# caishiqing/voice-tts

Measured on AMD Instinct MI355X. Metric: audio_seconds_per_second, higher is better.
Workload: dtype bf16

## Files before the change

### include/ixtts_hip.h

```cpp
#ifndef IXTTS_HIP_H
#define IXTTS_HIP_H

#include <stddef.h>
#include <stdint.h>

#ifdef __cplusplus
extern "C" {
#endif

#define IXTTS_OK 0
#define IXTTS_ERR_ARG (-1)
#define IXTTS_ERR_HIP (-2)
#define IXTTS_ERR_STATE (-3)
#define IXTTS_ERR_NOMEM (-4)
#define IXTTS_ERR_NAME (-5)

const char* ixtts_version(void);
const char* ixtts_last_error(void);

int ixtts_aa_snake_f32(const float* x_dev, float* y_dev, const float* up12_dev, const float* down12_dev,
                       const float* log_alpha_dev, const float* log_beta_dev, int B, int C, int T, void* stream);

size_t ixtts_attn_full_workspace_bytes(int B, int H, int T);
int ixtts_attn_full_f32(const float* q_dev, const float* k_dev, const float* v_dev, float* out_dev, int B, int H, int T,
                        int head_dim, long stride_b, long stride_t, long stride_h, long ostride_b, long ostride_t,
                        long ostride_h, float scale, void* workspace_dev, size_t workspace_bytes, void* stream);

int ixtts_adaln_rmsnorm_f32(const float* x_dev, const float* wb_dev, const float* g_dev, float* out_dev, int B, int T, int H, float eps,
                            void* stream);
int ixtts_ln_modulate_f32(const float* x_dev, const float* shift_scale_dev, float* out_dev, int B, int T, int H, float eps, void* stream);
int ixtts_rope_qk_f32(float* qkv_dev, const float* cos_sin_dev, int B, int T, int H, int head_dim, void* stream);
int ixtts_swiglu_f32(const float* u_dev, float* out_dev, long rows, int F, void* stream);
int ixtts_wn_gate_f32(const float* a_dev, const float* g_dev, float* out_dev, int B, int C, int T, long g_stride, int g_offset, void* stream);
int ixtts_wn_gate_rows_f32(const float* a_dev, const float* g_dev, float* out_dev, long rows, int C, long rows_per_batch, int B, long g_stride,
                           int g_offset, void* stream);
int ixtts_reflect_halo_rows_f32(float* p_dev, int B, int T, int C, int left, int right, void* stream);

size_t ixtts_gemm_x6_packed_bytes(int N, int K);
int ixtts_gemm_x6_pack(const float* w_dev, void* packed_dev, int N, int K, void* stream);
long ixtts_gemm_x6_rows_padded(long rows);
int ixtts_gemm_x6_split(const float* a_dev, long lda, void* planes_dev, long rows, int K, void* stream);
int ixtts_gemm_x6_f32(const void* a_planes_dev, long rows_total, long row0, const void* packed_dev, const float* bias_dev, float* c_dev, long ldc,
                      int M, int N, int K, int accumulate, int tile, void* stream);

#define IXTTS_BIGVGAN_MAX_STAGES 8
#define IXTTS_BIGVGAN_MAX_RESK 4

typedef struct ixtts_bigvgan_cfg {
  int num_mels;
  int upsample_initial_channel;
  int n_stages;
  int upsample_rates[IXTTS_BIGVGAN_MAX_STAGES];
  int upsample_kernel_sizes[IXTTS_BIGVGAN_MAX_STAGES];
  int n_resblock_kernels;
  int resblock_kernel_sizes[IXTTS_BIGVGAN_MAX_RESK];
  int resblock_dilations[IXTTS_BIGVGAN_MAX_RESK][3];
  int max_frames;
  int fast_sin;
} ixtts_bigvgan_cfg;

typedef struct ixtts_bigvgan ixtts_bigvgan;

int ixtts_bigvgan_create(ixtts_bigvgan** out, const ixtts_bigvgan_cfg* cfg);
int ixtts_bigvgan_set_tensor(ixtts_bigvgan* h, const char* name, const float* data_host, const int64_t* shape, int ndim);
int ixtts_bigvgan_finalize(ixtts_bigvgan* h);
int ixtts_bigvgan_arena(ixtts_bigvgan* h, void** ptr_dev, size_t* bytes);
int ixtts_bigvgan_adopt_arena(ixtts_bigvgan* h);
int ixtts_bigvgan_forward(ixtts_bigvgan* h, const float* mel_dev, int B, int F, float* wav_dev, void* stream);
double ixtts_bigvgan_flops(const ixtts_bigvgan* h, int B, int F);
int ixtts_bigvgan_destroy(ixtts_bigvgan* h);

#define IXTTS_DTYPE_F32 0
#define IXTTS_DTYPE_BF16 1

typedef struct ixtts_gpt_cfg {
  int model_dim;
// ... 69 lines not shown
```

### voice-tts_amd/_lib.py

```python
import ctypes as C
import os

HERE = os.path.dirname(os.path.abspath(__file__))
LIB_PATH = os.environ.get("IXTTS_LIB") or os.path.join(HERE, "libixtts_hip.so")

MAX_STAGES = 8
MAX_RESK = 4


class BigVGANCfg(C.Structure):
    _fields_ = [
        ("num_mels", C.c_int), ("upsample_initial_channel", C.c_int), ("n_stages", C.c_int),
        ("upsample_rates", C.c_int * MAX_STAGES), ("upsample_kernel_sizes", C.c_int * MAX_STAGES),
        ("n_resblock_kernels", C.c_int), ("resblock_kernel_sizes", C.c_int * MAX_RESK),
        ("resblock_dilations", (C.c_int * 3) * MAX_RESK), ("max_frames", C.c_int), ("fast_sin", C.c_int),
    ]


class GptCfg(C.Structure):
    _fields_ = [
        ("model_dim", C.c_int), ("layers", C.c_int), ("heads", C.c_int), ("n_mel_codes", C.c_int),
        ("n_mel_pos", C.c_int), ("n_text_tokens", C.c_int), ("n_text_pos", C.c_int),
        ("start_mel_token", C.c_int), ("stop_mel_token", C.c_int), ("max_seq", C.c_int),
        ("max_batch", C.c_int), ("weight_dtype", C.c_int),
    ]


class SamplerCfg(C.Structure):
    _fields_ = [
        ("repetition_penalty", C.c_float), ("temperature", C.c_float), ("top_k", C.c_int),
        ("top_p", C.c_float), ("do_sample", C.c_int), ("suppress_stop", C.c_int), ("seed", C.c_uint64),
        ("typical_mass", C.c_float), ("length_penalty", C.c_float),
    ]


_P = C.c_void_p
SYMBOLS = {
    "ixtts_version": (C.c_char_p, []),
    "ixtts_last_error": (C.c_char_p, []),
    "ixtts_aa_snake_f32": (C.c_int, [_P, _P, _P, _P, _P, _P, C.c_int, C.c_int, C.c_int, _P]),
    "ixtts_attn_full_workspace_bytes": (C.c_size_t, [C.c_int, C.c_int, C.c_int]),
    "ixtts_attn_full_f32": (C.c_int, [_P, _P, _P, _P, C.c_int, C.c_int, C.c_int, C.c_int, C.c_long, C.c_long, C.c_long, C.c_long, C.c_long,
                                      C.c_long, C.c_float, _P, C.c_size_t, _P]),
    "ixtts_adaln_rmsnorm_f32": (C.c_int, [_P, _P, _P, _P, C.c_int, C.c_int, C.c_int, C.c_float, _P]),
    "ixtts_ln_modulate_f32": (C.c_int, [_P, _P, _P, C.c_int, C.c_int, C.c_int, C.c_float, _P]),
    "ixtts_rope_qk_f32": (C.c_int, [_P, _P, C.c_int, C.c_int, C.c_int, C.c_int, _P]),
    "ixtts_swiglu_f32": (C.c_int, [_P, _P, C.c_long, C.c_int, _P]),
    "ixtts_wn_gate_f32": (C.c_int, [_P, _P, _P, C.c_int, C.c_int, C.c_int, C.c_long, C.c_int, _P]),
    "ixtts_wn_gate_rows_f32": (C.c_int, [_P, _P, _P, C.c_long, C.c_int, C.c_long, C.c_int, C.c_long, C.c_int, _P]),
    "ixtts_reflect_halo_rows_f32": (C.c_int, [_P, C.c_int, C.c_int, C.c_int, C.c_int, C.c_int, _P]),
    "ixtts_gemm_x6_packed_bytes": (C.c_size_t, [C.c_int, C.c_int]),
    "ixtts_gemm_x6_pack": (C.c_int, [_P, _P, C.c_int, C.c_int, _P]),
    "ixtts_gemm_x6_rows_padded": (C.c_long, [C.c_long]),
    "ixtts_gemm_x6_split": (C.c_int, [_P, C.c_long, _P, C.c_long, C.c_int, _P]),
    "ixtts_gemm_x6_f32": (C.c_int, [_P, C.c_long, C.c_long, _P, _P, _P, C.c_long, C.c_int, C.c_int, C.c_int, C.c_int, C.c_int, _P]),
    "ixtts_bigvgan_create": (C.c_int, [C.POINTER(_P), C.POINTER(BigVGANCfg)]),
    "ixtts_bigvgan_set_tensor": (C.c_int, [_P, C.c_char_p, _P, C.POINTER(C.c_int64), C.c_int]),
    "ixtts_bigvgan_finalize": (C.c_int, [_P]),
    "ixtts_bigvgan_arena": (C.c_int, [_P, C.POINTER(_P), C.POINTER(C.c_size_t)]),
    "ixtts_bigvgan_adopt_arena": (C.c_int, [_P]),
    "ixtts_bigvgan_forward": (C.c_int, [_P, _P, C.c_int, C.c_int, _P, _P]),
    "ixtts_bigvgan_flops": (C.c_double, [_P, C.c_int, C.c_int]),
    "ixtts_bigvgan_destroy": (C.c_int, [_P]),
    "ixtts_gpt_create": (C.c_int, [C.POINTER(_P), C.POINTER(GptCfg)]),
    "ixtts_gpt_set_tensor": (C.c_int, [_P, C.c_char_p, _P, C.POINTER(C.c_int64), C.c_int]),
    "ixtts_gpt_finalize": (C.c_int, [_P]),
    "ixtts_gpt_arena": (C.c_int, [_P, C.POINTER(_P), C.POINTER(C.c_size_t)]),
    "ixtts_gpt_adopt_arena": (C.c_int, [_P]),
    "ixtts_gpt_share_arena": (C.c_int, [_P, _P]),
    "ixtts_gpt_prefill": (C.c_int, [_P, C.c_int, _P, C.c_int, C.c_int, _P]),
    "ixtts_gpt_decode": (C.c_int, [_P, C.c_int, C.c_int, C.POINTER(SamplerCfg), _P]),
    "ixtts_gpt_read": (C.c_int, [_P, C.c_int, _P, C.c_int, C.POINTER(C.c_int), C.POINTER(C.c_int), _P]),
    "ixtts_gpt_read_logits": (C.c_int, [_P, C.c_int, _P, _P]),
    "ixtts_gpt_beam_begin": (C.c_int, [_P, C.c_int, _P]),
    "ixtts_gpt_beam_decode": (C.c_int, [_P, C.c_int, C.POINTER(SamplerCfg), _P]),
    "ixtts_gpt_beam_read": (C.c_int, [_P, C.c_int, _P, C.c_int, C.POINTER(C.c_int), C.POINTER(C.c_int), C.POINTER(C.c_float), _P, _P, _P, _P]),
    "ixtts_gpt_beam_force": (C.c_int, [_P, _P, C.c_int, _P]),
    "ixtts_gpt_beam_begin_group": (C.c_int, [_P, C.c_int, C.c_int, C.c_uint64, _P]),
    "ixtts_gpt_beam_park_group": (C.c_int, [_P, C.c_int, _P]),
    "ixtts_gpt_beam_decode_groups": (C.c_int, [_P, C.c_int, C.c_int, C.POINTER(SamplerCfg), _P]),
    "ixtts_gpt_beam_read_group": (C.c_int, [_P, C.c_int, C.c_int, _P, C.c_int, C.POINTER(C.c_int), C.POINTER(C.c_int), C.POINTER(C.c_float), _P, _P, _P, _P]),
    "ixtts_gpt_beam_force_group": (C.c_int, [_P, C.c_int, _P, C.c_int, _P]),
    "ixtts_gpt_read_probs": (C.c_int, [_P, C.c_int, _P, _P]),
    "ixtts_gpt_force_next": (C.c_int, [_P, C.c_int, C.c_int32, _P]),
    "ixtts_gpt_latent": (C.c_int, [_P, _P, C.c_int, _P, C.c_int, _P, _P]),
    "ixtts_gpt_bench_gemv": (C.c_int, [_P, C.c_int, C.c_int, C.c_int, _P]),
    "ixtts_gpt_step_bytes": (C.c_double, [_P, C.c_int, C.c_int]),
    "ixtts_gpt_max_batch": (C.c_int, []),
# ... 44 lines not shown
```

### voice-tts_amd/csrc/gemm_x6.hip

```cpp
#include "common.h"

namespace ixtts {

typedef float gx_f32x16 __attribute__((ext_vector_type(16)));
typedef __bf16 gx_bf16x8 __attribute__((ext_vector_type(8)));
typedef float gx_f32x4 __attribute__((ext_vector_type(4)));
typedef unsigned int gx_u32x4 __attribute__((ext_vector_type(4)));


__global__ void gemm_x6_pack_kernel(const float* __restrict__ w, uint4* __restrict__ out, int N, int K, int Npad) {
  const long total = (long)(K / 8) * Npad;
  for (long idx = blockIdx.x * (long)blockDim.x + threadIdx.x; idx < total; idx += (long)gridDim.x * blockDim.x) {
    const int n = (int)(idx % Npad);
    const int ko = (int)(idx / Npad);
    float v[8];
#pragma unroll
    for (int e = 0; e < 8; ++e) v[e] = n < N ? w[(long)n * K + ko * 8 + e] : 0.f;
    uint4 ph, pm, pl;
    split8_bf16x3(v, ph, pm, pl);
    const int g = ko >> 1, kh = ko & 1;
    uint4* base = out + ((long)g * 6) * Npad + n;
    base[(long)(0 * 2 + kh) * Npad] = ph;
    base[(long)(1 * 2 + kh) * Npad] = pm;
    base[(long)(2 * 2 + kh) * Npad] = pl;
  }
}

__global__ __launch_bounds__(256) void gemm_x6_split_kernel(const float* __restrict__ a, long lda, uint4* __restrict__ out, int M, int K, long Mpad) {
  __shared__ float tile[64][65];
  const int r0 = blockIdx.x * 64, k0 = blockIdx.y * 64;
  const int t = threadIdx.x;
#pragma unroll
  for (int i = 0; i < 4; ++i) {
    const int r = (t >> 4) + 16 * i, kq = t & 15;
    float4 v = make_float4(0.f, 0.f, 0.f, 0.f);
    if (r0 + r < M) v = *reinterpret_cast<const float4*>(a + (long)(r0 + r) * lda + k0 + 4 * kq);
    tile[r][4 * kq + 0] = v.x; tile[r][4 * kq + 1] = v.y; tile[r][4 * kq + 2] = v.z; tile[r][4 * kq + 3] = v.w;
  }
  __syncthreads();
#pragma unroll
  for (int u = 0; u < 2; ++u) {
    const int r = t & 63, o = (t >> 6) + 4 * u;
    float v[8];
#pragma unroll
    for (int e = 0; e < 8; ++e) v[e] = tile[r][o * 8 + e];
    uint4 ph, pm, pl;
    split8_bf16x3(v, ph, pm, pl);
    const int ko = (k0 >> 3) + o, g = ko >> 1, kh = ko & 1;
    uint4* base = out + ((long)g * 6) * Mpad + r0 + r;
    base[(long)(0 * 2 + kh) * Mpad] = ph;
    base[(long)(1 * 2 + kh) * Mpad] = pm;
    base[(long)(2 * 2 + kh) * Mpad] = pl;
  }
}

struct GemmX6Params {
  const uint4* Ap;
  long Mpad;
  long arow0;
  const uint4* Wp;
  const float* bias;
  float* C;
  long ldc;
  int M, N, Npad, K, accumulate, m_tiles, n_tiles;
  unsigned long long* dbg;
};


template <int MT, int NT, int NST, int DBG = 0>
__global__ __launch_bounds__(256, (NST * (MT + NT) * 6 * 64 * 16 <= 80 * 1024) ? 2 : 1) void gemm_x6_kernel(GemmX6Params p) {
  constexpr int BM = 64 * MT, BN = 64 * NT;
  constexpr int A_UNITS = 6 * BM, W_UNITS = 6 * BN, STAGE = A_UNITS + W_UNITS;
  constexpr int NDMA = (6 * (MT + NT)) / 4;
  static_assert((6 * (MT + NT)) % 4 == 0, "the copies are dealt evenly to the 4 waves");
  constexpr int D = NST - 1;
  extern __shared__ uint4 smem[];

  const int nwg = p.m_tiles * p.n_tiles;
  const int bid = blockIdx.x;
  const int xcd = bid & 7, idx = bid >> 3;
  const int qd = nwg >> 3, rm = nwg & 7;
  const int lin = (xcd < rm ? xcd * (qd + 1) : rm * (qd + 1) + (xcd - rm) * qd) + idx;
  const int m_tile = lin / p.n_tiles, n_tile = lin - m_tile * p.n_tiles;
  const int m0 = m_tile * BM, n0 = n_tile * BN;

  const int tid = threadIdx.x, lane = tid & 63, wave = tid >> 6;
  const int wm = wave >> 1, wn = wave & 1;
  const int l31 = lane & 31, lh = lane >> 5;

  gx_f32x16 acc[MT][NT];
#pragma unroll
  for (int i = 0; i < MT; ++i)
#pragma unroll
    for (int j = 0; j < NT; ++j)
#pragma unroll
      for (int r = 0; r < 16; ++r) acc[i][j][r] = 0.f;

  const uint4* asrc = p.Ap + p.arow0 + m0 + lane;
  const uint4* wsrc = p.Wp + n0 + lane;
  auto issue = [&](int s, uint4* st) {
#pragma unroll
    for (int q = 0; q < NDMA; ++q) {
      const int e = q * 4 + wave;
      if (e < 6 * MT) {
        const int run = e / MT, piece = e % MT;
        __builtin_amdgcn_global_load_lds((const __attribute__((address_space(1))) void*)(asrc + ((long)s * 6 + run) * p.Mpad + piece * 64),
                                         (__attribute__((address_space(3))) void*)(st + run * BM + piece * 64), 16, 0, 0);
      } else {
        const int e2 = e - 6 * MT, run = e2 / NT, piece = e2 % NT;
        __builtin_amdgcn_global_load_lds((const __attribute__((address_space(1))) void*)(wsrc + ((long)s * 6 + run) * p.Npad + piece * 64),
                                         (__attribute__((address_space(3))) void*)(st + A_UNITS + run * BN + piece * 64), 16, 0, 0);
      }
    }
  };

  const int steps = p.K >> 4;
  auto wg_stamp = [&](int k) {
    if constexpr (DBG == 3) {
      if (tid == 0) p.dbg[128 + (long)blockIdx.x * 4 + k] = __builtin_amdgcn_s_memrealtime();
    }
  };
  auto wait_younger = [&](int y) {
    if (y >= 2) asm volatile("s_waitcnt vmcnt(%0)" ::"n"(2 * NDMA) : "memory");
    else if (y == 1) asm volatile("s_waitcnt vmcnt(%0)" ::"n"(NDMA) : "memory");
    else asm volatile("s_waitcnt vmcnt(0)" ::: "memory");
  };
  static_assert(D >= 1 && D <= 3, "1..3 steps of copies in flight behind the one waited for");
  wg_stamp(0);
  for (int t = 0; t < D && t < steps; ++t) issue(t, smem + t * STAGE);
  wait_younger(min(D, steps) - 1);
  __builtin_amdgcn_s_barrier();
  asm volatile("" ::: "memory");
  wg_stamp(1);

  const unsigned base_addr = (unsigned)(uintptr_t)(const __attribute__((address_space(3))) void*)smem;
  int st_cur = 0, st_nxt = D % NST;
  for (int s = 0; s < steps; ++s) {
    auto stamp = [&](int k) {
      if constexpr (DBG == 3) {
// ... 37 lines not shown
              "=&v"(bf[1][0]), "=&v"(bf[1][1]), "=&v"(bf[2][0]), "=&v"(bf[2][1])
            : "v"(aaddr), "v"(waddr), "n"((0 * 2 * BM + 0) * 16), "n"((0 * 2 * BM + 32) * 16), "n"((1 * 2 * BM + 0) * 16), "n"((1 * 2 * BM + 32) * 16),
              "n"((2 * 2 * BM + 0) * 16), "n"((2 * 2 * BM + 32) * 16), "n"((0 * 2 * BN + 0) * 16), "n"((0 * 2 * BN + 32) * 16), "n"((1 * 2 * BN + 0) * 16),
              "n"((1 * 2 * BN + 32) * 16), "n"((2 * 2 * BN + 0) * 16), "n"((2 * 2 * BN + 32) * 16)
            : "memory");
      }
      stamp(2);
#pragma unroll
      for (int i = 0; i < MT; ++i)
#pragma unroll
        for (int j = 0; j < NT; ++j) {
          const gx_bf16x8 ah = __builtin_bit_cast(gx_bf16x8, af[0][i]), am = __builtin_bit_cast(gx_bf16x8, af[1][i]), al = __builtin_bit_cast(gx_bf16x8, af[2][i]);
          const gx_bf16x8 bh = __builtin_bit_cast(gx_bf16x8, bf[0][j]), bm = __builtin_bit_cast(gx_bf16x8, bf[1][j]), bl = __builtin_bit_cast(gx_bf16x8, bf[2][j]);
          acc[i][j] = __builtin_amdgcn_mfma_f32_32x32x16_bf16(al, bh, acc[i][j], 0, 0, 0);
          acc[i][j] = __builtin_amdgcn_mfma_f32_32x32x16_bf16(ah, bl, acc[i][j], 0, 0, 0);
          acc[i][j] = __builtin_amdgcn_mfma_f32_32x32x16_bf16(am, bm, acc[i][j], 0, 0, 0);
          acc[i][j] = __builtin_amdgcn_mfma_f32_32x32x16_bf16(am, bh, acc[i][j], 0, 0, 0);
          acc[i][j] = __builtin_amdgcn_mfma_f32_32x32x16_bf16(ah, bm, acc[i][j], 0, 0, 0);
          acc[i][j] = __builtin_amdgcn_mfma_f32_32x32x16_bf16(ah, bh, acc[i][j], 0, 0, 0);
        }
      if constexpr (DBG == 3) asm volatile("" ::"v"(acc[0][0][0]), "v"(acc[MT - 1][NT - 1][15]));
    }
    stamp(3);
    wait_younger(DBG == 1 ? 0 : max(0, min(D - 1, steps - s - 2)));
    stamp(4);
    __builtin_amdgcn_s_barrier();
    asm volatile("" ::: "memory");
    stamp(5);
    st_cur = st_cur + 1 == NST ? 0 : st_cur + 1;
    st_nxt = st_nxt + 1 == NST ? 0 : st_nxt + 1;
  }

  wg_stamp(2);
#pragma unroll
  for (int j = 0; j < NT; ++j) {
    const int col = n0 + wn * (32 * NT) + j * 32 + l31;
    const bool col_ok = col < p.N;
    const float bv = (p.bias != nullptr && col_ok) ? p.bias[col] : 0.f;
#pragma unroll
    for (int i = 0; i < MT; ++i) {
      const int rbase = m0 + wm * (32 * MT) + i * 32 + 4 * lh;
#pragma unroll
      for (int r = 0; r < 16; ++r) {
        const int row = rbase + (r & 3) + 8 * (r >> 2);
        if (col_ok && row < p.M) {
          float* c = p.C + (long)row * p.ldc + col;
          float v = acc[i][j][r] + bv;
          if (p.accumulate) v += *c;
          *c = v;
        }
      }
    }
  }
  if constexpr (DBG == 3) {
    asm volatile("s_waitcnt vmcnt(0)" ::: "memory");
    wg_stamp(3);
  }
}

template <int MT, int NT, int NST, int DBG = 0>
static int launch_gemm_x6(GemmX6Params p, hipStream_t st) {
  constexpr int BM = 64 * MT, BN = 64 * NT;
  constexpr size_t smem = (size_t)NST * (6 * BM + 6 * BN) * 16;
  static_assert(smem <= 160 * 1024, "LDS stages of this tile shape");
  p.m_tiles = ceil_div(p.M, BM);
  p.n_tiles = ceil_div(p.N, BN);
  IX_ARG((long)p.n_tiles * BN <= p.Npad, "gemm_x6: packed weights padded to %d features, the %d-wide tile needs %d", p.Npad, BN, p.n_tiles * BN);
  IX_ARG(p.arow0 + (long)p.m_tiles * BM <= p.Mpad, "gemm_x6: activation planes hold %ld rows, the %d-row tiles reach row %ld", p.Mpad, BM, p.arow0 + (long)p.m_tiles * BM);
  auto kern = gemm_x6_kernel<MT, NT, NST, DBG>;
  static bool done = false;
  if (!done) {
    IX_HIP(hipFuncSetAttribute((const void*)kern, hipFuncAttributeMaxDynamicSharedMemorySize, (int)smem));
    done = true;
  }
  hipLaunchKernelGGL(kern, dim3(p.m_tiles * p.n_tiles), dim3(256), smem, st, p);
  IX_HIP(hipGetLastError());
  return IXTTS_OK;
}

}

using namespace ixtts;

extern "C" size_t ixtts_gemm_x6_packed_bytes(int N, int K) {
  if (N <= 0 || K <= 0 || K % 64) return 0;
  const size_t Npad = (size_t)(N + 255) / 256 * 256;
  return (size_t)(K / 16) * 6 * Npad * 16;
}

extern "C" int ixtts_gemm_x6_pack(const float* w_dev, void* packed_dev, int N, int K, void* stream) {
  IX_ARG(w_dev && packed_dev && N > 0 && K > 0 && K % 64 == 0, "gemm_x6_pack: bad argument (K must be a multiple of 64)");
  const int Npad = (N + 255) / 256 * 256;
  const long total = (long)(K / 8) * Npad;
  hipLaunchKernelGGL(gemm_x6_pack_kernel, dim3((unsigned)std::min<long>((total + 255) / 256, 4096)), dim3(256), 0, (hipStream_t)stream, w_dev,
                     reinterpret_cast<uint4*>(packed_dev), N, K, Npad);
  IX_HIP(hipGetLastError());
  return IXTTS_OK;
}

extern "C" long ixtts_gemm_x6_rows_padded(long rows) { return rows <= 0 ? 0 : (rows + 255) / 256 * 256 + 256; }

extern "C" int ixtts_gemm_x6_split(const float* a_dev, long lda, void* planes_dev, long rows, int K, void* stream) {
  IX_ARG(a_dev && planes_dev && rows > 0 && K > 0 && K % 64 == 0, "gemm_x6_split: bad argument (K must be a multiple of 64)");
  IX_ARG(lda >= K && lda % 4 == 0 && (reinterpret_cast<uintptr_t>(a_dev) & 15) == 0, "gemm_x6_split: rows must be 16-byte aligned (lda %ld)", lda);
  const long Mpad = ixtts_gemm_x6_rows_padded(rows);
  hipLaunchKernelGGL(gemm_x6_split_kernel, dim3((unsigned)(Mpad / 64), K / 64), dim3(256), 0, (hipStream_t)stream, a_dev, lda,
                     reinterpret_cast<uint4*>(planes_dev), (int)rows, K, Mpad);
  IX_HIP(hipGetLastError());
  return IXTTS_OK;
}

extern "C" int ixtts_gemm_x6_f32(const void* a_planes_dev, long rows_total, long row0, const void* packed_dev, const float* bias_dev, float* c_dev,
                                 long ldc, int M, int N, int K, int accumulate, int tile, void* stream) {
  IX_ARG(a_planes_dev && packed_dev && c_dev && M > 0 && N > 0 && K > 0 && K % 64 == 0, "gemm_x6: bad argument (K must be a multiple of 64: the split pass works on 64-wide k blocks)");
  IX_ARG(ldc >= N && row0 >= 0 && row0 + M <= rows_total, "gemm_x6: rows [%ld, %ld) of %ld, ldc %ld", row0, row0 + M, rows_total, ldc);
  GemmX6Params p;
  p.Ap = reinterpret_cast<const uint4*>(a_planes_dev); p.Mpad = ixtts_gemm_x6_rows_padded(rows_total); p.arow0 = row0;
  p.Wp = reinterpret_cast<const uint4*>(packed_dev); p.bias = bias_dev; p.C = c_dev; p.ldc = ldc;
  p.M = M; p.N = N; p.Npad = (N + 255) / 256 * 256; p.K = K; p.accumulate = accumulate ? 1 : 0; p.m_tiles = p.n_tiles = 0;
  p.dbg = (tile == 32 || tile == 33) ? reinterpret_cast<unsigned long long*>(const_cast<float*>(bias_dev)) : nullptr;
  if (p.dbg) p.bias = nullptr;
  hipStream_t st = (hipStream_t)stream;
  if (tile == 0) {
    const long t42 = (long)ceil_div(M, 256) * ceil_div(N, 128);
    tile = t42 >= 140 ? 2 : 3;
  }
  switch (tile) {
    case 2: return launch_gemm_x6<4, 2, 2>(p, st);
    case 3: return launch_gemm_x6<2, 2, 3>(p, st);
    case 4: return launch_gemm_x6<4, 2, 4>(p, st);
    case 5: return launch_gemm_x6<2, 2, 4>(p, st);
    case 12: return launch_gemm_x6<4, 2, 2, 1>(p, st);
    case 22: return launch_gemm_x6<4, 2, 2, 2>(p, st);
    case 32: return launch_gemm_x6<4, 2, 2, 3>(p, st);
    case 33: return launch_gemm_x6<2, 2, 3, 3>(p, st);
  }
  set_error("gemm_x6: tile %d (0 auto; 2 / 3: 256x128 / 128x128, two workgroups per CU; 4 / 5: the same, one per CU with a 4-stage ring)", tile);
  return IXTTS_ERR_ARG;
}
```

### voice-tts_amd/gemm.py

```python
import ctypes as C

import torch

from . import _lib


class PackedLinear:

    __slots__ = ("N", "K", "packed", "bias")

    def __init__(self, weight, bias=None):
        assert weight.is_cuda and weight.dim() == 2 and weight.shape[1] % 64 == 0, tuple(weight.shape)
        w = weight.detach().to(torch.float32).contiguous()
        self.N, self.K = int(w.shape[0]), int(w.shape[1])
        nbytes = _lib.lib().ixtts_gemm_x6_packed_bytes(self.N, self.K)
        self.packed = torch.empty(nbytes, dtype=torch.uint8, device=w.device)
        with torch.cuda.device(w.device):
            _lib.check(_lib.lib().ixtts_gemm_x6_pack(w.data_ptr(), self.packed.data_ptr(), self.N, self.K, _lib.current_stream_ptr()), "ixtts_gemm_x6_pack")
            torch.cuda.current_stream().synchronize()
        self.bias = None if bias is None else bias.detach().to(w.device, torch.float32).contiguous()


class Planes:

# ... 15 lines not shown
    K = int(x.shape[-1])
    if x.dim() != 2:
        x = x.reshape(-1, K) if x.is_contiguous() else x.contiguous().reshape(-1, K)
    rows, lda = int(x.shape[0]), int(x.stride(0))
    L = _lib.lib()
    nbytes = (K // 16) * 6 * int(L.ixtts_gemm_x6_rows_padded(rows)) * 16
    key = (x.device, nbytes, slot)
    buf = _POOL.get(key)
    if buf is None:
        buf = _POOL[key] = torch.empty(nbytes, dtype=torch.uint8, device=x.device)
    with torch.cuda.device(x.device):
        _lib.check(L.ixtts_gemm_x6_split(x.data_ptr(), lda, buf.data_ptr(), rows, K, _lib.current_stream_ptr()), "ixtts_gemm_x6_split")
    return Planes(buf, rows, K)


def linear(x, pl, out=None, accumulate=False, bias=True, tile=0, row0=0, rows=None, lead=None):
    K, N = pl.K, pl.N
    if not isinstance(x, Planes):
        lead = tuple(x.shape[:-1]) if lead is None else lead
        x = split(x)
    assert x.K == K, (x.K, K)
    M = (x.rows - row0) if rows is None else int(rows)
    if out is None:
        assert not accumulate
        out = torch.empty(*(lead if lead is not None else (M,)), N, dtype=torch.float32, device=pl.packed.device)
    assert out.shape[-1] == N and out.stride(-1) == 1 and out.numel() >= M * N
    ldc = int(out.stride(-2)) if out.dim() >= 2 else N
    b = pl.bias if (bias and pl.bias is not None) else None
    with torch.cuda.device(pl.packed.device):
        rc = _lib.lib().ixtts_gemm_x6_f32(x.buf.data_ptr(), x.rows, int(row0), pl.packed.data_ptr(), b.data_ptr() if b is not None else None, out.data_ptr(), ldc,
                                          M, N, K, 1 if accumulate else 0, int(tile), _lib.current_stream_ptr())
    _lib.check(rc, "ixtts_gemm_x6_f32")
    return out
```

### voice-tts_amd/s2mel.py

```python
import math
import os

import torch
import torch.nn.functional as F

from .convs import conv1d

from .weights import fold_weight_norm

S2MEL_CFG = dict(
    hidden_dim=512, num_heads=8, depth=13, in_channels=80, content_dim=512, style_dim=192,
    wavenet_hidden=512, wavenet_layers=8, wavenet_kernel=5, wavenet_dilation_rate=1,
    lr_channels=512, lr_in_channels=1024, lr_n_blocks=4, gpt_dim=1280, codebook_dim=8, codebook_size=8192, semantic_dim=1024,
)


def tiny_s2mel_cfg(**kw):
    c = dict(S2MEL_CFG)
    c.update(hidden_dim=64, num_heads=2, depth=5, content_dim=32, style_dim=12, wavenet_hidden=64, wavenet_layers=3,
             lr_channels=32, lr_in_channels=40, lr_n_blocks=2, gpt_dim=128, codebook_size=8194, semantic_dim=40)
    c.update(kw)
    return c


def _ffn_dim(dim):
    n_hidden = int(2 * (4 * dim) / 3)
    return n_hidden if n_hidden % 256 == 0 else n_hidden + 256 - (n_hidden % 256)


def s2mel_shapes(cfg=S2MEL_CFG):
    H, Hw, C = cfg["hidden_dim"], cfg["wavenet_hidden"], cfg["in_channels"]
    assert H == Hw, "FinalLayer's adaLN takes the DiT timestep embedding: wavenet.hidden_dim must equal DiT.hidden_dim"
    out = [("gpt_layer.0.weight", (256, cfg["gpt_dim"])), ("gpt_layer.0.bias", (256,)), ("gpt_layer.1.weight", (128, 256)),
           ("gpt_layer.1.bias", (128,)), ("gpt_layer.2.weight", (cfg["semantic_dim"], 128)), ("gpt_layer.2.bias", (cfg["semantic_dim"],)),
           ("quantizer.codebook.weight", (cfg["codebook_size"], cfg["codebook_dim"])),
           ("quantizer.out_project.weight", (cfg["semantic_dim"], cfg["codebook_dim"], 1)), ("quantizer.out_project.bias", (cfg["semantic_dim"],))]
    lr = cfg["lr_channels"]
    out += [("length_regulator.content_in_proj.weight", (lr, cfg["lr_in_channels"])), ("length_regulator.content_in_proj.bias", (lr,))]
# ... 241 lines not shown
        self.t_freqs = torch.exp(-math.log(10000.0) * torch.arange(half, dtype=torch.float32) / half).to(self.device)
        self._rope = None
        W, C_, L = self.W, cfg["in_channels"], cfg["depth"]
        t = "cfm.estimator.transformer."
        self.w13 = [torch.cat([W[t + f"layers.{i}.feed_forward.w1.weight"], W[t + f"layers.{i}.feed_forward.w3.weight"]], 0).contiguous() for i in range(L)]
        self.skip_w = {i: (W[t + f"layers.{i}.skip_in_linear.weight"][:, :H].contiguous(), W[t + f"layers.{i}.skip_in_linear.weight"][:, H:].contiguous())
                       for i in range(L // 2 + 1, L)}
        names = [t + f"layers.{i}.{n}" for i in range(L) for n in ("attention_norm", "ffn_norm")] + [t + "norm"]
        self.proj_w = torch.cat([W[n + ".project_layer.weight"] for n in names], 0).contiguous()
        self.proj_b = torch.cat([W[n + ".project_layer.bias"] for n in names], 0).contiguous()
        mw = W["cfm.estimator.cond_x_merge_linear.weight"]
        self.merge_x, self.merge_rest = mw[:, :C_].contiguous(), mw[:, C_:].contiguous()
        wn = "cfm.estimator.wavenet."
        self.wn_taps = [[W[wn + f"in_layers.{i}.conv.conv.weight"][:, :, j].contiguous() for j in range(cfg["wavenet_kernel"])]
                        for i in range(cfg["wavenet_layers"])]
        nl, Hw = cfg["wavenet_layers"], cfg["wavenet_hidden"]
        self.wn_r1, self.wn_r2, self.wn_bin = [], [], []
        carry = torch.zeros(Hw, device=self.device)
        self.wn_out_bias = torch.zeros(Hw, device=self.device)
        for i in range(nl):
            rw, rb = W[wn + f"res_skip_layers.{i}.conv.conv.weight"][:, :, 0], W[wn + f"res_skip_layers.{i}.conv.conv.bias"]
            self.wn_bin.append(W[wn + f"in_layers.{i}.conv.conv.bias"] + sum(self.wn_taps[i]) @ carry)
            if i < nl - 1:
                self.wn_r1.append(rw[:Hw].contiguous())
                self.wn_r2.append(rw[Hw:].contiguous())
                carry = carry + rb[:Hw]
                self.wn_out_bias = self.wn_out_bias + rb[Hw:]
            else:
                self.wn_r1.append(None)
                self.wn_r2.append(rw.contiguous())
                self.wn_out_bias = self.wn_out_bias + rb
        sw = W["cfm.estimator.skip_linear.weight"]
        self.skipl_res, self.skipl_x = sw[:, :H].contiguous(), sw[:, H:].contiguous()

    def gpt_layer(self, latent):
        x = _lin(latent, self.W, "gpt_layer.0")
        x = _lin(x, self.W, "gpt_layer.1")
        return _lin(x, self.W, "gpt_layer.2")

    def vq2emb(self, codes):
        emb = self.W["quantizer.codebook.weight"][codes.long()]
        out = conv1d(emb.transpose(1, 2), self.W["quantizer.out_project.weight"], self.W["quantizer.out_project.bias"])
        return out.transpose(1, 2)

    def length_regulator(self, x, ylens):
        W = self.W
        x = _lin(x, W, "length_regulator.content_in_proj")
        T = int(ylens.max())
        x = F.interpolate(x.transpose(1, 2).contiguous(), size=T, mode="nearest")
        for i in range(self.cfg["lr_n_blocks"]):
            x = conv1d(x, W[f"length_regulator.model.{3 * i}.weight"], W[f"length_regulator.model.{3 * i}.bias"], padding=1)
            x = F.group_norm(x, 1, W[f"length_regulator.model.{3 * i + 1}.weight"], W[f"length_regulator.model.{3 * i + 1}.bias"], 1e-5)
            x = F.mish(x)
        n = 3 * self.cfg["lr_n_blocks"]
        x = conv1d(x, W[f"length_regulator.model.{n}.weight"], W[f"length_regulator.model.{n}.bias"])
        mask = (torch.arange(T, device=x.device).unsqueeze(0) < ylens.unsqueeze(1)).unsqueeze(-1)
        return x.transpose(1, 2) * mask

    def _t_embed(self, t, prefix):
        args = 1000.0 * t[:, None].float() * self.t_freqs[None]
        emb = torch.cat([torch.cos(args), torch.sin(args)], dim=-1)
        h = F.silu(_lin(emb, self.W, prefix + ".mlp.0"))
        return _lin(h, self.W, prefix + ".mlp.2")

    def _rope_cache(self, T):
        if self._rope is None or self._rope.shape[0] < T:
            n = self.head_dim
            freqs = 1.0 / (10000.0 ** (torch.arange(0, n, 2)[: n // 2].float() / n))
            ang = torch.outer(torch.arange(max(T, 64)).float(), freqs)
            self._rope = torch.polar(torch.ones_like(ang), ang).to(self.device)
        return self._rope[:T]

    @staticmethod
    def _rotary(x, fc):
        xc = torch.view_as_complex(x.reshape(*x.shape[:-1], -1, 2))
        return torch.view_as_real(xc * fc.view(1, fc.shape[0], 1, fc.shape[1])).flatten(3)

    def _attention(self, qkv, B, T, mask):
        H, nh, hd = self.cfg["hidden_dim"], self.cfg["num_heads"], self.head_dim
        fc = self._rope_cache(T)
        if mask is None and hd == 64 and qkv.is_cuda:
            with torch.cuda.device(qkv.device):
                _hip_call("ixtts_rope_qk_f32", qkv.data_ptr(), torch.view_as_real(fc).data_ptr(), B, T, H, hd)
            v4 = qkv.view(B, T, 3, nh, hd)
            return attn_full(v4[:, :, 0], v4[:, :, 1], v4[:, :, 2]).reshape(B * T, H)
        q, k, v = qkv.view(B, T, 3 * H).split([H, H, H], dim=-1)
        q = self._rotary(q.reshape(B, T, nh, hd), fc)
        k = self._rotary(k.reshape(B, T, nh, hd), fc)
        v = v.reshape(B, T, nh, hd)
        y = F.scaled_dot_product_attention(q.transpose(1, 2), k.transpose(1, 2), v.transpose(1, 2), attn_mask=mask, dropout_p=0.0)
        return y.transpose(1, 2).reshape(B * T, H)

    def _transformer(self, x, c, mask):
        W, cfg = self.W, self.cfg
        B, T, H = x.shape
        L = cfg["depth"]
        wb_all = F.linear(c, self.proj_w, self.proj_b).view(B, 2 * L + 1, 2 * H).transpose(0, 1).contiguous()
        x = x.reshape(B * T, H)
        skips = []
        for i in range(L):
            p = f"cfm.estimator.transformer.layers.{i}."
            if i > L // 2:
                wa, wb_ = self.skip_w[i]
                x = F.linear(skips.pop(), wb_, W[p + "skip_in_linear.bias"]).addmm_(x, wa.t())
            a = adaln_rmsnorm(x.view(B, T, H), wb_all[2 * i], W[p + "attention_norm.norm.weight"])
            y = self._attention(F.linear(a.view(B * T, H), W[p + "attention.wqkv.weight"]), B, T, mask)
            h = torch.addmm(x, y, W[p + "attention.wo.weight"].t()) if 0 < i <= L // 2 else x.addmm_(y, W[p + "attention.wo.weight"].t())
            f = adaln_rmsnorm(h.view(B, T, H), wb_all[2 * i + 1], W[p + "ffn_norm.norm.weight"])
            x = h.addmm_(swiglu(F.linear(f.view(B * T, H), self.w13[i])), W[p + "feed_forward.w2.weight"].t())
            if i < L // 2:
                skips.append(x)
        return adaln_rmsnorm(x.view(B, T, H), wb_all[2 * L], W["cfm.estimator.transformer.norm.norm.weight"])

    def _wavenet(self, x, x_mask, g, full):
        W, cfg = self.W, self.cfg
        Hw, nl, k = cfg["wavenet_hidden"], cfg["wavenet_layers"], cfg["wavenet_kernel"]
        p = "cfm.estimator.wavenet."
        g = F.linear(g, W[p + "cond_layer.conv.conv.weight"][:, :, 0], W[p + "cond_layer.conv.conv.bias"])
        out = None
        for i in range(nl):
            d = cfg["wavenet_dilation_rate"] ** i
            tot = (k - 1) * d
            right = tot // 2
            xin = _pad_reflect(x, tot - right, right)
            if x.is_cuda:
                wk, T_ = self.wn_taps[i], x.shape[-1]
                acc = W[p + f"in_layers.{i}.conv.conv.bias"][None, :, None].expand(x.shape[0], -1, T_)
                for j in range(k):
                    wj, xj = wk[j].expand(x.shape[0], -1, -1), xin[:, :, j * d:j * d + T_]
                    acc = torch.baddbmm(acc, wj, xj) if j == 0 else acc.baddbmm_(wj, xj)
                xin = acc
            else:
                xin = conv1d(xin, W[p + f"in_layers.{i}.conv.conv.weight"], W[p + f"in_layers.{i}.conv.conv.bias"], dilation=d)
            acts = wn_gate(xin, g, i * 2 * Hw, Hw)
            rs = conv1d(acts, W[p + f"res_skip_layers.{i}.conv.conv.weight"], W[p + f"res_skip_layers.{i}.conv.conv.bias"])
            if i < nl - 1:
                x = x + rs[:, :Hw]
                if not full:
                    x = x * x_mask
                out = rs[:, Hw:] if out is None else out + rs[:, Hw:]
            else:
                out = rs if out is None else out + rs
# ... 10 lines not shown
        for i in range(nl):
            d = cfg["wavenet_dilation_rate"] ** i
            tot = (k - 1) * d
            right = tot // 2
            xin = _pad_reflect(x, tot - right, right)
            acc = self.wn_bin[i][None, :, None].expand(B, -1, T_)
            for j in range(k):
                wj, xj = self.wn_taps[i][j].expand(B, -1, -1), xin[:, :, j * d:j * d + T_]
                acc = torch.baddbmm(acc, wj, xj) if j == 0 else acc.baddbmm_(wj, xj)
            acts = wn_gate(acc, g, i * 2 * Hw, Hw)
            if i < nl - 1:
                x = x.baddbmm_(self.wn_r1[i].expand(B, -1, -1), acts)
            r2 = self.wn_r2[i].expand(B, -1, -1)
            out = torch.bmm(r2, acts) if out is None else out.baddbmm_(r2, acts)
        return out

    def _wavenet_rows(self, h, g):
        W, cfg = self.W, self.cfg
        Hw, nl, k = cfg["wavenet_hidden"], cfg["wavenet_layers"], cfg["wavenet_kernel"]
        assert cfg["wavenet_dilation_rate"] == 1
        B, T_, _ = h.shape
        p = "cfm.estimator.wavenet."
        g = F.linear(g, W[p + "cond_layer.conv.conv.weight"][:, :, 0], W[p + "cond_layer.conv.conv.bias"])
        tot = k - 1
        right = tot // 2
        left = tot - right
        Tp = T_ + tot
        P = torch.empty(B, Tp, Hw, device=h.device, dtype=h.dtype)
        P[:, left:left + T_] = h
        P2 = P.view(B * Tp, Hw)
        M = B * Tp - tot
        centre = P2[left:left + M]
        out = torch.empty(B * Tp, Hw, device=h.device, dtype=h.dtype)
        for i in range(nl):
            reflect_halo_rows(P, T_, left, right)
            acc = torch.addmm(self.wn_bin[i], P2[:M], self.wn_taps[i][0].t())
            for j in range(1, k):
                acc.addmm_(P2[j:j + M], self.wn_taps[i][j].t())
            acts = wn_gate_rows(acc, g, i * 2 * Hw, Hw, Tp)
            if i < nl - 1:
                centre.addmm_(acts, self.wn_r1[i].t())
            if i == 0:
                torch.mm(acts, self.wn_r2[i].t(), out=out[:M])
            else:
                out[:M].addmm_(acts, self.wn_r2[i].t())
        return out.view(B, Tp, Hw)[:, :T_]

    def dit_prepare(self, prompt_x, x_lens, style, cond):
        W = self.W
        e = "cfm.estimator."
        B, _, T = prompt_x.shape
        cond = _lin(cond, W, e + "cond_projection")
        rest = torch.cat([prompt_x.transpose(1, 2), cond, style[:, None, :].expand(B, T, style.shape[-1])], dim=-1)
        base = F.linear(rest, self.merge_rest, W[e + "cond_x_merge_linear.bias"])
        x_mask = (torch.arange(T, device=prompt_x.device).unsqueeze(0) < x_lens.unsqueeze(1)).unsqueeze(1)
        full = int(x_lens.min()) >= T
        if full:
            attn_mask = None
        else:
            attn_mask = x_mask[:, None, :].expand(x_mask.shape[0], 1, T, T)
            if attn_mask.shape[0] != B:
                attn_mask = attn_mask.expand(B, 1, T, T)
        return dict(B=B, T=T, base=base, x_mask=x_mask.to(base.dtype), attn_mask=attn_mask, full=full)

    def dit_step(self, ctx, x, t, out_from=0):
        W, cfg = self.W, self.cfg
        e = "cfm.estimator."
        B, T, base = ctx["B"], ctx["T"], ctx["base"]
        xt = x.transpose(1, 2)
        t1 = self._t_embed(t, e + "t_embedder")
        x_in = base + F.linear(xt, self.merge_x)
        x_res = self._transformer(x_in, t1, ctx["attn_mask"])
# ... 72 lines not shown
```

Before: 39.80.

## Fuse SwiGLU and WaveNet gate epilogues into x6 GEMM with tap-shifted conv

Adds a paired-output GEMM path to the x6 kernel. Weight halves are interleaved in 32-column blocks so each wave holds both halves, letting the kernel apply a SwiGLU or tanh·sigmoid gate epilogue in-register and write only the half-width result. The WaveNet dilated conv is folded into one GEMM: each k-tap reads the activation planes shifted by a row offset instead of issuing k separate addmm calls. This removes the intermediate full-width tensor, the separate activation kernels and the extra GEMM launches. The cost is an extra split pass on the inputs, and the epilogue uses expf/tanhf per element.

```diff
diff --git a/include/ixtts_hip.h b/include/ixtts_hip.h
--- a/include/ixtts_hip.h
+++ b/include/ixtts_hip.h
@@ -42,6 +42,9 @@
 int ixtts_gemm_x6_split(const float* a_dev, long lda, void* planes_dev, long rows, int K, void* stream);
 int ixtts_gemm_x6_f32(const void* a_planes_dev, long rows_total, long row0, const void* packed_dev, const float* bias_dev, float* c_dev, long ldc,
                       int M, int N, int K, int accumulate, int tile, void* stream);
+int ixtts_gemm_x6_pair_f32(const void* a_planes_dev, long rows_total, long row0, int taps, const void* packed_dev, const float* bias_dev,
+                           const float* gate_dev, long gate_ld, long rows_per_batch, int nbatch, float* c_dev, long ldc, int M, int N, int K,
+                           int epilogue, int tile, void* stream);
 
 #define IXTTS_BIGVGAN_MAX_STAGES 8
 #define IXTTS_BIGVGAN_MAX_RESK 4
diff --git a/voice-tts_amd/_lib.py b/voice-tts_amd/_lib.py
--- a/voice-tts_amd/_lib.py
+++ b/voice-tts_amd/_lib.py
@@ -54,6 +54,8 @@
     "ixtts_gemm_x6_rows_padded": (C.c_long, [C.c_long]),
     "ixtts_gemm_x6_split": (C.c_int, [_P, C.c_long, _P, C.c_long, C.c_int, _P]),
     "ixtts_gemm_x6_f32": (C.c_int, [_P, C.c_long, C.c_long, _P, _P, _P, C.c_long, C.c_int, C.c_int, C.c_int, C.c_int, C.c_int, _P]),
+    "ixtts_gemm_x6_pair_f32": (C.c_int, [_P, C.c_long, C.c_long, C.c_int, _P, _P, _P, C.c_long, C.c_long, C.c_int, _P, C.c_long, C.c_int, C.c_int,
+                                         C.c_int, C.c_int, C.c_int, _P]),
     "ixtts_bigvgan_create": (C.c_int, [C.POINTER(_P), C.POINTER(BigVGANCfg)]),
     "ixtts_bigvgan_set_tensor": (C.c_int, [_P, C.c_char_p, _P, C.POINTER(C.c_int64), C.c_int]),
     "ixtts_bigvgan_finalize": (C.c_int, [_P]),
diff --git a/voice-tts_amd/csrc/gemm_x6.hip b/voice-tts_amd/csrc/gemm_x6.hip
--- a/voice-tts_amd/csrc/gemm_x6.hip
+++ b/voice-tts_amd/csrc/gemm_x6.hip
@@ -53,6 +53,8 @@
     base[(long)(2 * 2 + kh) * Mpad] = pl;
   }
 }
+
+enum { EPI_PLAIN = 0, EPI_SWIGLU = 1, EPI_GATE = 2 };
 
 struct GemmX6Params {
   const uint4* Ap;
@@ -63,6 +65,11 @@
   float* C;
   long ldc;
   int M, N, Npad, K, accumulate, m_tiles, n_tiles;
+  int tap_steps;
+  int epi;
+  const float* gate;
+  long gate_ld, rows_per_batch;
+  int nbatch;
   unsigned long long* dbg;
 };
 
@@ -99,12 +106,13 @@
   const uint4* asrc = p.Ap + p.arow0 + m0 + lane;
   const uint4* wsrc = p.Wp + n0 + lane;
   auto issue = [&](int s, uint4* st) {
+    const int tap = s / p.tap_steps, sa = s - tap * p.tap_steps;
 #pragma unroll
     for (int q = 0; q < NDMA; ++q) {
       const int e = q * 4 + wave;
       if (e < 6 * MT) {
         const int run = e / MT, piece = e % MT;
-        __builtin_amdgcn_global_load_lds((const __attribute__((address_space(1))) void*)(asrc + ((long)s * 6 + run) * p.Mpad + piece * 64),
+        __builtin_amdgcn_global_load_lds((const __attribute__((address_space(1))) void*)(asrc + ((long)sa * 6 + run) * p.Mpad + tap + piece * 64),
                                          (__attribute__((address_space(3))) void*)(st + run * BM + piece * 64), 16, 0, 0);
       } else {
         const int e2 = e - 6 * MT, run = e2 / NT, piece = e2 % NT;
@@ -208,6 +216,34 @@
   }
 
   wg_stamp(2);
+  if (p.epi != EPI_PLAIN) {
+    static_assert(NT == 2, "pair epilogues: the wave's two 32-column blocks are the two halves");
+    const int oc = (n0 + wn * 64) / 2 + l31;
+    const int nh = p.N >> 1;
+    if (oc < nh) {
+      const float ba = p.bias != nullptr ? p.bias[n0 + wn * 64 + l31] : 0.f, bb = p.bias != nullptr ? p.bias[n0 + wn * 64 + 32 + l31] : 0.f;
+#pragma unroll
+      for (int i = 0; i < MT; ++i) {
+        const int rbase = m0 + wm * (32 * MT) + i * 32 + 4 * lh;
+#pragma unroll
+        for (int r = 0; r < 16; ++r) {
+          const int row = rbase + (r & 3) + 8 * (r >> 2);
+          if (row < p.M) {
+            float a = acc[i][0][r] + ba, b = acc[i][1][r] + bb, v;
+            if (p.epi == EPI_SWIGLU) {
+              v = a / (1.0f + expf(-a)) * b;
+            } else {
+              const float* g = p.gate + (long)min((long)row / p.rows_per_batch, (long)p.nbatch - 1) * p.gate_ld;
+              a += g[oc];
+              b += g[nh + oc];
+              v = tanhf(a) * (1.0f / (1.0f + expf(-b)));
+            }
+            p.C[(long)row * p.ldc + oc] = v;
+          }
+        }
+      }
+    }
+  } else
 #pragma unroll
   for (int j = 0; j < NT; ++j) {
     const int col = n0 + wn * (32 * NT) + j * 32 + l31;
@@ -242,7 +278,9 @@
   p.m_tiles = ceil_div(p.M, BM);
   p.n_tiles = ceil_div(p.N, BN);
   IX_ARG((long)p.n_tiles * BN <= p.Npad, "gemm_x6: packed weights padded to %d features, the %d-wide tile needs %d", p.Npad, BN, p.n_tiles * BN);
-  IX_ARG(p.arow0 + (long)p.m_tiles * BM <= p.Mpad, "gemm_x6: activation planes hold %ld rows, the %d-row tiles reach row %ld", p.Mpad, BM, p.arow0 + (long)p.m_tiles * BM);
+  const int taps = (p.K >> 4) / p.tap_steps;
+  IX_ARG(p.arow0 + (long)p.m_tiles * BM + taps - 1 <= p.Mpad, "gemm_x6: activation planes hold %ld rows, the %d-row tiles reach row %ld", p.Mpad, BM,
+         p.arow0 + (long)p.m_tiles * BM + taps - 1);
   auto kern = gemm_x6_kernel<MT, NT, NST, DBG>;
   static bool done = false;
   if (!done) {
@@ -286,19 +324,9 @@
   return IXTTS_OK;
 }
 
-extern "C" int ixtts_gemm_x6_f32(const void* a_planes_dev, long rows_total, long row0, const void* packed_dev, const float* bias_dev, float* c_dev,
-                                 long ldc, int M, int N, int K, int accumulate, int tile, void* stream) {
-  IX_ARG(a_planes_dev && packed_dev && c_dev && M > 0 && N > 0 && K > 0 && K % 64 == 0, "gemm_x6: bad argument (K must be a multiple of 64: the split pass works on 64-wide k blocks)");
-  IX_ARG(ldc >= N && row0 >= 0 && row0 + M <= rows_total, "gemm_x6: rows [%ld, %ld) of %ld, ldc %ld", row0, row0 + M, rows_total, ldc);
-  GemmX6Params p;
-  p.Ap = reinterpret_cast<const uint4*>(a_planes_dev); p.Mpad = ixtts_gemm_x6_rows_padded(rows_total); p.arow0 = row0;
-  p.Wp = reinterpret_cast<const uint4*>(packed_dev); p.bias = bias_dev; p.C = c_dev; p.ldc = ldc;
-  p.M = M; p.N = N; p.Npad = (N + 255) / 256 * 256; p.K = K; p.accumulate = accumulate ? 1 : 0; p.m_tiles = p.n_tiles = 0;
-  p.dbg = (tile == 32 || tile == 33) ? reinterpret_cast<unsigned long long*>(const_cast<float*>(bias_dev)) : nullptr;
-  if (p.dbg) p.bias = nullptr;
-  hipStream_t st = (hipStream_t)stream;
+static int run_gemm_x6(GemmX6Params p, int tile, hipStream_t st) {
   if (tile == 0) {
-    const long t42 = (long)ceil_div(M, 256) * ceil_div(N, 128);
+    const long t42 = (long)ceil_div(p.M, 256) * ceil_div(p.N, 128);
     tile = t42 >= 140 ? 2 : 3;
   }
   switch (tile) {
@@ -314,3 +342,36 @@
   set_error("gemm_x6: tile %d (0 auto; 2 / 3: 256x128 / 128x128, two workgroups per CU; 4 / 5: the same, one per CU with a 4-stage ring)", tile);
   return IXTTS_ERR_ARG;
 }
+
+extern "C" int ixtts_gemm_x6_f32(const void* a_planes_dev, long rows_total, long row0, const void* packed_dev, const float* bias_dev, float* c_dev,
+                                 long ldc, int M, int N, int K, int accumulate, int tile, void* stream) {
+  IX_ARG(a_planes_dev && packed_dev && c_dev && M > 0 && N > 0 && K > 0 && K % 64 == 0, "gemm_x6: bad argument (K must be a multiple of 64: the split pass works on 64-wide k blocks)");
+  IX_ARG(ldc >= N && row0 >= 0 && row0 + M <= rows_total, "gemm_x6: rows [%ld, %ld) of %ld, ldc %ld", row0, row0 + M, rows_total, ldc);
+  GemmX6Params p;
+  p.Ap = reinterpret_cast<const uint4*>(a_planes_dev); p.Mpad = ixtts_gemm_x6_rows_padded(rows_total); p.arow0 = row0;
+  p.Wp = reinterpret_cast<const uint4*>(packed_dev); p.bias = bias_dev; p.C = c_dev; p.ldc = ldc;
+  p.M = M; p.N = N; p.Npad = (N + 255) / 256 * 256; p.K = K; p.accumulate = accumulate ? 1 : 0; p.m_tiles = p.n_tiles = 0;
+  p.tap_steps = K >> 4; p.epi = EPI_PLAIN; p.gate = nullptr; p.gate_ld = 0; p.rows_per_batch = 1; p.nbatch = 1;
+  p.dbg = (tile == 32 || tile == 33) ? reinterpret_cast<unsigned long long*>(const_cast<float*>(bias_dev)) : nullptr;
+  if (p.dbg) p.bias = nullptr;
+  return run_gemm_x6(p, tile, (hipStream_t)stream);
+}
+
+extern "C" int ixtts_gemm_x6_pair_f32(const void* a_planes_dev, long rows_total, long row0, int taps, const void* packed_dev, const float* bias_dev,
+                                      const float* gate_dev, long gate_ld, long rows_per_batch, int nbatch, float* c_dev, long ldc, int M, int N, int K,
+                                      int epilogue, int tile, void* stream) {
+  IX_ARG(a_planes_dev && packed_dev && c_dev && M > 0 && N > 0 && taps > 0 && K > 0, "gemm_x6_pair: bad argument");
+  IX_ARG(K % taps == 0 && (K / taps) % 64 == 0 && N % 64 == 0, "gemm_x6_pair: K %d = %d taps of a multiple of 64, N %d a multiple of 64", K, taps, N);
+  IX_ARG(epilogue == EPI_SWIGLU || (epilogue == EPI_GATE && gate_dev && rows_per_batch > 0 && nbatch > 0 && gate_ld >= N / 2),
+         "gemm_x6_pair: epilogue %d (1 swiglu; 2 gate, with gate biases)", epilogue);
+  IX_ARG(ldc >= N / 2 && row0 >= 0 && row0 + M + taps - 1 <= rows_total, "gemm_x6_pair: rows [%ld, %ld) + %d taps of %ld, ldc %ld", row0, row0 + M, taps,
+         rows_total, ldc);
+  IX_ARG(tile == 0 || tile == 2 || tile == 3, "gemm_x6_pair: tile %d (0 auto, 2, 3)", tile);
+  GemmX6Params p;
+  p.Ap = reinterpret_cast<const uint4*>(a_planes_dev); p.Mpad = ixtts_gemm_x6_rows_padded(rows_total); p.arow0 = row0;
+  p.Wp = reinterpret_cast<const uint4*>(packed_dev); p.bias = bias_dev; p.C = c_dev; p.ldc = ldc;
+  p.M = M; p.N = N; p.Npad = (N + 255) / 256 * 256; p.K = K; p.accumulate = 0; p.m_tiles = p.n_tiles = 0;
+  p.tap_steps = (K / taps) >> 4; p.epi = epilogue; p.gate = gate_dev; p.gate_ld = gate_ld; p.rows_per_batch = rows_per_batch; p.nbatch = nbatch;
+  p.dbg = nullptr;
+  return run_gemm_x6(p, tile, (hipStream_t)stream);
+}
diff --git a/voice-tts_amd/gemm.py b/voice-tts_amd/gemm.py
--- a/voice-tts_amd/gemm.py
+++ b/voice-tts_amd/gemm.py
@@ -71,3 +71,34 @@
                                           M, N, K, 1 if accumulate else 0, int(tile), _lib.current_stream_ptr())
     _lib.check(rc, "ixtts_gemm_x6_f32")
     return out
+
+
+SWIGLU, GATE = 1, 2
+
+
+def interleave_halves(a, b):
+    F = a.shape[0]
+    assert b.shape == a.shape and F % 32 == 0, (tuple(a.shape), tuple(b.shape))
+    return torch.stack([a.reshape(F // 32, 32, *a.shape[1:]), b.reshape(F // 32, 32, *b.shape[1:])], 1).reshape(2 * F, *a.shape[1:]).contiguous()
+
+
+def pair_linear(x, pl, epilogue, taps=1, out=None, gate=None, gate_off=0, rows_per_batch=1, row0=0, rows=None, tile=0):
+    if not isinstance(x, Planes):
+        x = split(x)
+    assert pl.K == taps * x.K and pl.N % 64 == 0, (pl.K, taps, x.K, pl.N)
+    M = (x.rows - row0 - (taps - 1)) if rows is None else int(rows)
+    if out is None:
+        out = torch.empty(M, pl.N // 2, dtype=torch.float32, device=pl.packed.device)
+    assert out.shape[-1] == pl.N // 2 and out.stride(-1) == 1 and out.numel() >= M * (pl.N // 2)
+    ldc = int(out.stride(-2)) if out.dim() >= 2 else pl.N // 2
+    gp, gld, nb = None, 0, 1
+    if epilogue == GATE:
+        assert gate.is_contiguous() and gate.dim() == 2 and gate_off + pl.N <= gate.shape[1]
+        gp, gld, nb = gate.data_ptr() + 4 * int(gate_off), int(gate.shape[1]), int(gate.shape[0])
+    b = pl.bias
+    with torch.cuda.device(pl.packed.device):
+        rc = _lib.lib().ixtts_gemm_x6_pair_f32(x.buf.data_ptr(), x.rows, int(row0), int(taps), pl.packed.data_ptr(), b.data_ptr() if b is not None else None,
+                                               gp, gld, int(rows_per_batch), nb, out.data_ptr(), ldc, M, pl.N, pl.K, int(epilogue), int(tile),
+                                               _lib.current_stream_ptr())
+    _lib.check(rc, "ixtts_gemm_x6_pair_f32")
+    return out
diff --git a/voice-tts_amd/s2mel.py b/voice-tts_amd/s2mel.py
--- a/voice-tts_amd/s2mel.py
+++ b/voice-tts_amd/s2mel.py
@@ -4,6 +4,7 @@
 import torch
 import torch.nn.functional as F
 
+from . import gemm as G
 from .convs import conv1d
 
 from .weights import fold_weight_norm
@@ -311,6 +312,15 @@
                 self.wn_out_bias = self.wn_out_bias + rb
         sw = W["cfm.estimator.skip_linear.weight"]
         self.skipl_res, self.skipl_x = sw[:, :H].contiguous(), sw[:, H:].contiguous()
+        self.x6_w13, self.x6_wn = None, None
+        if self.device.type == "cuda" and H % 64 == 0:
+            inter = self.w13[0].shape[0] // 2
+            self.x6_w13 = [G.PackedLinear(G.interleave_halves(w[:inter], w[inter:])) for w in self.w13]
+            self.x6_wn = [G.PackedLinear(G.interleave_halves(torch.cat(tp, 1)[:Hw], torch.cat(tp, 1)[Hw:]), G.interleave_halves(b[:Hw], b[Hw:]))
+                          for tp, b in zip(self.wn_taps, self.wn_bin)]
+
+    def _x6(self, packs):
+        return packs is not None and os.environ.get("IXTTS_S2MEL_GEMM", "x6") != "library"
 
     def gpt_layer(self, latent):
         x = _lin(latent, self.W, "gpt_layer.0")
@@ -376,6 +386,7 @@
         L = cfg["depth"]
         wb_all = F.linear(c, self.proj_w, self.proj_b).view(B, 2 * L + 1, 2 * H).transpose(0, 1).contiguous()
         x = x.reshape(B * T, H)
+        x6 = x.is_cuda and self._x6(self.x6_w13)
         skips = []
         for i in range(L):
             p = f"cfm.estimator.transformer.layers.{i}."
@@ -385,8 +396,9 @@
             a = adaln_rmsnorm(x.view(B, T, H), wb_all[2 * i], W[p + "attention_norm.norm.weight"])
             y = self._attention(F.linear(a.view(B * T, H), W[p + "attention.wqkv.weight"]), B, T, mask)
             h = torch.addmm(x, y, W[p + "attention.wo.weight"].t()) if 0 < i <= L // 2 else x.addmm_(y, W[p + "attention.wo.weight"].t())
-            f = adaln_rmsnorm(h.view(B, T, H), wb_all[2 * i + 1], W[p + "ffn_norm.norm.weight"])
-            x = h.addmm_(swiglu(F.linear(f.view(B * T, H), self.w13[i])), W[p + "feed_forward.w2.weight"].t())
+            f = adaln_rmsnorm(h.view(B, T, H), wb_all[2 * i + 1], W[p + "ffn_norm.norm.weight"]).view(B * T, H)
+            u = G.pair_linear(f, self.x6_w13[i], G.SWIGLU) if x6 else swiglu(F.linear(f, self.w13[i]))
+            x = h.addmm_(u, W[p + "feed_forward.w2.weight"].t())
             if i < L // 2:
                 skips.append(x)
         return adaln_rmsnorm(x.view(B, T, H), wb_all[2 * L], W["cfm.estimator.transformer.norm.norm.weight"])
@@ -463,12 +475,16 @@
         M = B * Tp - tot
         centre = P2[left:left + M]
         out = torch.empty(B * Tp, Hw, device=h.device, dtype=h.dtype)
+        x6 = self._x6(self.x6_wn)
         for i in range(nl):
             reflect_halo_rows(P, T_, left, right)
-            acc = torch.addmm(self.wn_bin[i], P2[:M], self.wn_taps[i][0].t())
-            for j in range(1, k):
-                acc.addmm_(P2[j:j + M], self.wn_taps[i][j].t())
-            acts = wn_gate_rows(acc, g, i * 2 * Hw, Hw, Tp)
+            if x6:
+                acts = G.pair_linear(G.split(P2), self.x6_wn[i], G.GATE, taps=k, gate=g, gate_off=i * 2 * Hw, rows_per_batch=Tp)
+            else:
+                acc = torch.addmm(self.wn_bin[i], P2[:M], self.wn_taps[i][0].t())
+                for j in range(1, k):
+                    acc.addmm_(P2[j:j + M], self.wn_taps[i][j].t())
+                acts = wn_gate_rows(acc, g, i * 2 * Hw, Hw, Tp)
             if i < nl - 1:
                 centre.addmm_(acts, self.wn_r1[i].t())
             if i == 0:
```

After: 40.56 (median of 6 runs). 1.9% higher.
